# genome-vendor/bsmap

Hardware: AMD Instinct MI355X
Metric: aligned reads/sec (whole node), 2x150 bp hg38 WGBS -v 6 -s 16 (higher is better)
Workload: dtype u32; 1 GPU; C3: 2x150(->144) bp PE WGBS vs hg38-sized synthetic genome, -s 16 -v 6 -I 4 -m 28 -x 500; genome_bp=3088269832, index_entries=1475952693, parallelism=read-sharded x1, batches_in_flight=2, exact_mode=False, resident_ring_steps=4, records_flagged_BSX_F_LIMIT=0

## Files before the change

### bsmap_amd/csrc/bsx_align.hip

```cpp
#include "bsx_internal.h"
#include "bsx_dev.h"
#include "bsx_kernel_args.h"

namespace {

typedef unsigned long long u64;

struct __attribute__((packed, aligned(4))) U4 { uint32_t a, b, c, d; };
struct __attribute__((packed, aligned(4))) U2 { uint32_t a, b; };

#ifndef BSX_MAIN_NT
#define BSX_MAIN_NT 0
#endif
#ifndef BSX_MAIN_PREFETCH
#define BSX_MAIN_PREFETCH 1
#endif
typedef uint32_t v4u_a4 __attribute__((ext_vector_type(4), aligned(4)));
typedef uint32_t v2u_a4 __attribute__((ext_vector_type(2), aligned(4)));
__device__ __forceinline__ U4 ldm4(const uint32_t *p)
{
#if BSX_MAIN_NT
    const v4u_a4 v = __builtin_nontemporal_load(reinterpret_cast<const v4u_a4 *>(p));
    return U4{v.x, v.y, v.z, v.w};
#else
// ... 2199 lines not shown
    __shared__ uint32_t TAB[BSX_HSCAN_WPB][4][32];
    __shared__ uint2 PT[BSX_HSCAN_WPB][HP_PAIRS * 32];
    __shared__ uint2 QBUF[BSX_HSCAN_WPB][HP_QCAP];
    const int lane = threadIdx.x & 63, wv = (int)rfl(threadIdx.x >> 6);
    const uint32_t n_tasks = min(*H.n_tasks, H.task_cap);
    const uint32_t nvb = (n_tasks + BSX_HSCAN_WPB - 1) / BSX_HSCAN_WPB;
    for (uint32_t vb = blockIdx.x;; vb += gridDim.x) {
        uint32_t b_;
        const int st_ = bsx_order_block(vb, nvb, H.xcd_map, b_);
        if (st_ == 2) break;
        if (st_ == 1) continue;
        const uint32_t slot = b_ * BSX_HSCAN_WPB + (uint32_t)wv;
        if (slot < n_tasks) hp_task<STATS>(A, H, H.order ? rfl(H.order[slot]) : slot, lane, TAB[wv], PT[wv], QBUF[wv]);
        wave_fence();
    }
}

#ifndef HG_WPB
#define HG_WPB 1
#endif
#ifndef HG_R
#define HG_R 64u
#endif
static_assert(HG_R == 16u || HG_R == 32u || HG_R == 48u || HG_R == 64u, "a lane per member: 64 at most, and whole quarters of a segment");
#ifndef HG_XCD_DIV
#define HG_XCD_DIV (HG_R > 16u ? 2u : 1u)
#endif
#ifndef HG_C
#define HG_C 4
#endif
#ifndef HG_BIG
#define HG_BIG (HG_R > 32u ? 33u : 1u)
#endif
#ifndef HG_PREFETCH
#define HG_PREFETCH 0
#endif
#ifndef HG_EXIT
#define HG_EXIT 15
#endif
#ifndef BSX_HSAME_WAVES
#define BSX_HSAME_WAVES 4
#endif
#ifndef HG_D
#define HG_D 2
#endif
#ifndef HG_ROWPF
#define HG_ROWPF 0
// ... 354 lines not shown
        uint32_t tid = 0, th = 0, tc0 = 0, tn = 0, key = 0, hh = 0, flags = 0, tx = 0, tw = 0;
        if ((uint32_t)lane < K) {
            tid = H.order[slot + lane];
            const HTask tk = H.tasks[tid];
            th = tk.h; tc0 = tk.c0; tn = tk.n; key = tk.key; hh = tk.sub_h; flags = tk.flags; tx = tk.pad[0]; tw = tk.pad[1];
        }
        const uint32_t n0 = rfl(tn), f0 = rfl(flags);
        if (n0 == 0) {
            if ((uint32_t)lane < K) { HTaskOut *o = &H.tout[tid]; o->count = 0; o->overflow = 0; o->acc[0] = o->acc[1] = o->acc[2] = o->acc[3] = 0; o->c0 = 0; o->n = 0; }
        } else if (f0 & 4u) {
            if (((f0 >> 8) & 15u) == 3u) hs_group<3, true, STATS>(A, H, L, lane, wv, K, tid, th, tc0, rfl(key), n0, rfl(hh), hh, f0, rfl(tx), rfl(tw));
            else hs_group<0, true, STATS>(A, H, L, lane, wv, K, tid, th, tc0, rfl(key), n0, rfl(hh), hh, f0, rfl(tx), rfl(tw));
        }
        else if (K > 1) {
            if (((f0 >> 8) & 15u) == 5u) hs_group<5, false, STATS>(A, H, L, lane, wv, K, tid, th, tc0, rfl(key), n0, rfl(hh), hh, f0, 0u, 0u);
            else if (((f0 >> 8) & 15u) == 4u) hs_group<4, false, STATS>(A, H, L, lane, wv, K, tid, th, tc0, rfl(key), n0, rfl(hh), hh, f0, 0u, 0u);
            else hs_group<0, false, STATS>(A, H, L, lane, wv, K, tid, th, tc0, rfl(key), n0, rfl(hh), hh, f0, 0u, 0u);
        }
        else hp_task<STATS>(A, H, rfl(tid), lane, L.W[wv].one.TAB, L.W[wv].one.PT, L.W[wv].one.Q);
        wave_fence();
    }
}

__global__ __launch_bounds__(256) void k_task_groups(const HTask *tasks, const uint32_t *n_tasks_ptr, uint32_t cap, uint32_t *order, uint32_t *ghead, uint32_t *glist, uint32_t D, uint32_t Rg)
{
    const int lane = threadIdx.x & 63;
    const uint32_t n_tasks = min(*n_tasks_ptr, cap);
    for (uint32_t s0 = (blockIdx.x * 4u + (threadIdx.x >> 6)) * 64u; s0 < n_tasks; s0 += gridDim.x * 256u) {
        const uint32_t nj = min(64u, n_tasks - s0);
        uint32_t tid = 0, tn = 0, key = 0, hh = 0, flags = 0, tx = 0, tw = 0;
        if ((uint32_t)lane < nj) {
            tid = order[s0 + lane];
            const HTask tk = tasks[tid];
            tn = tk.n; key = tk.key; hh = tk.sub_h; flags = tk.flags; tx = tk.pad[0]; tw = tk.pad[1];
        }
        u64 todo = bsx_ballot((uint32_t)lane < nj);
        uint32_t off = 0, head = 0, dst = 0;
        while (todo) {
            const uint32_t i0 = (uint32_t)__builtin_ctzll(todo);
            const uint32_t n0 = rl_u(tn, i0), f0 = rl_u(flags, i0), key0 = rl_u(key, i0), h0 = rl_u(hh, i0), tx0 = rl_u(tx, i0), tw0 = rl_u(tw, i0);
            const bool pending = (todo >> lane) & 1;
            u64 mem = 1ull << i0;
            if (n0 == 0) mem = bsx_ballot(pending && tn == 0);
            else if (f0 & 2u) {
                const uint32_t Dg = (!(f0 & 4u) && ((f0 >> 8) & 15u) == 5u) ? D : 0u;
                const bool win = pending && tn == n0 && key == key0 && flags == f0 && tx == tx0 && tw == tw0;
                uint32_t hmin = h0;
                if (Dg) {
                    uint32_t v = win && ((hh ^ h0) & 31u) == 0 ? hh ^ 0x80000000u : 0xffffffffu;
#pragma unroll
                    for (int o = 32; o; o >>= 1) v = min(v, (uint32_t)__shfl_xor(v, o));
                    hmin = v ^ 0x80000000u;
                }
                const uint32_t dh = hh - hmin;
                mem = 0;
                uint32_t Kg = 0;
                for (uint32_t dd = 0; dd <= Dg && Kg < Rg; dd++) {
                    const bool same = win && dh == 32u * dd;
                    u64 md = bsx_ballot(same);
                    if (Kg + (uint32_t)__builtin_popcountll(md) > Rg) md = bsx_ballot(same && Kg + (uint32_t)__builtin_popcountll(md & lanemask_lt(lane)) < Rg);
                    if ((md >> lane) & 1) dst = off + Kg + (uint32_t)__builtin_popcountll(md & lanemask_lt(lane));
                    mem |= md; Kg += (uint32_t)__builtin_popcountll(md);
                }
            }
            const uint32_t K = (uint32_t)__builtin_popcountll(mem);
            if (!(n0 != 0 && (f0 & 2u)) && ((mem >> lane) & 1)) dst = off + (uint32_t)__builtin_popcountll(mem & lanemask_lt(lane));
            if ((uint32_t)lane == off) head = K;
            off += K; todo &= ~mem;
        }
        if ((uint32_t)lane < nj) { order[s0 + dst] = tid; ghead[s0 + lane] = head; }
        const u64 hb = bsx_ballot(head >= HG_BIG), hs = bsx_ballot(head != 0 && head < HG_BIG);
        uint32_t base = 0;
        if (lane == 0 && hb) base = atomicAdd(&glist[cap], (uint32_t)__builtin_popcountll(hb));
        if (lane == 1 && hs) base = atomicAdd(&glist[cap + 1], (uint32_t)__builtin_popcountll(hs));
        const uint32_t base_b = rl_u(base, 0), base_s = rl_u(base, 1);
        if (head >= HG_BIG) glist[base_b + (uint32_t)__builtin_popcountll(hb & lanemask_lt(lane))] = s0 + (uint32_t)lane;
        else if (head != 0) glist[cap - 1u - (base_s + (uint32_t)__builtin_popcountll(hs & lanemask_lt(lane)))] = s0 + (uint32_t)lane;
    }
}

#define HS_SHARE 16u
#ifndef BSX_HSHARED_W3
#define BSX_HSHARED_W3 1
#endif
#ifndef BSX_HSHARED_C2
#define BSX_HSHARED_C2 1
#endif
#ifndef BSX_HSHARED_WAVES
#define BSX_HSHARED_WAVES 5
#endif
struct SharedChunk { uint32_t wd[12]; uint32_t pm1, strand; bool valid; };

__device__ __forceinline__ U2 shared_entry(const U2 *__restrict__ ent2, uint32_t idx, bool in_range)
{
    U2 e; e.a = 0xFFFFFFFFu; e.b = 0;
    if (in_range) e = ent2[idx];
    return e;
}
template <int NWR, bool LDS_CHR>
__device__ __forceinline__ SharedChunk shared_gather(const U2 e, bool in_range, uint32_t h, uint32_t tag_xor, uint32_t tag_want, const uint32_t *anch_lds,
// ... 390 lines not shown
}
__global__ __launch_bounds__(256) void k_task_order(const HTask *tasks, const uint32_t *n_tasks_ptr, uint32_t cap, uint32_t shift, uint32_t n_bins, uint32_t spread, const uint32_t *bstart,
                                                     const uint32_t *chunk_tot, uint32_t n_chunks, const uint32_t *rank, uint32_t *order)
{
    __shared__ uint32_t cstart[1024];
    const uint32_t n = min(*n_tasks_ptr, cap);
    if (n == 0) return;
    for (uint32_t i = threadIdx.x; i < 1024; i += 256) cstart[i] = i < n_chunks ? chunk_tot[i] : 0u;
    __syncthreads();
    for (uint32_t o = 1; o < 1024; o <<= 1) {
        uint32_t t[4];
        for (int k = 0; k < 4; k++) { const uint32_t i = threadIdx.x + 256 * k; t[k] = i >= o ? cstart[i - o] : 0u; }
        __syncthreads();
        for (int k = 0; k < 4; k++) cstart[threadIdx.x + 256 * k] += t[k];
        __syncthreads();
    }
    for (uint32_t i = blockIdx.x * 256 + threadIdx.x; i < n; i += gridDim.x * 256) {
        const uint32_t b = task_bin(tasks[i], shift, n_bins, spread), c = b / BIN_CHUNK;
        order[(c ? cstart[c - 1] : 0u) + bstart[b] + rank[i]] = i;
    }
}
}

uint32_t bsx_bin_chunks(uint32_t n_bins) { return (n_bins + BIN_CHUNK - 1) / BIN_CHUNK; }

void bsx_launch_task_order(const HeavyArgsRaw &R, uint32_t shift, uint32_t n_bins, uint32_t *bins, uint32_t *bstart, uint32_t *chunk_tot, uint32_t *rank, uint32_t *order,
                           uint32_t *zero_blk, hipStream_t stream, uint32_t spread, bool groups, uint32_t same_d, uint32_t same_r)
{
    const uint32_t grid = std::max(1u, std::min(512u, (R.task_cap + 255u) / 256u)), n_chunks = bsx_bin_chunks(n_bins);
    hipLaunchKernelGGL(k_task_bins, dim3(std::max(1u, std::min(256u, (R.task_cap + 1023u) / 1024u))), dim3(256), 0, stream, (const HTask *)R.tasks, R.n_tasks, R.task_cap, shift, n_bins, spread, bins, rank, zero_blk);
    hipLaunchKernelGGL(k_bin_scan, dim3(n_chunks), dim3(256), 0, stream, R.n_tasks, bins, bstart, chunk_tot, n_bins, groups ? R.glist + R.task_cap : (uint32_t *)nullptr);
    hipLaunchKernelGGL(k_task_order, dim3(grid), dim3(256), 0, stream, (const HTask *)R.tasks, R.n_tasks, R.task_cap, shift, n_bins, spread, bstart, chunk_tot, n_chunks, rank, order);
    if (groups) hipLaunchKernelGGL(k_task_groups, dim3(std::max(1u, std::min(1024u, (R.task_cap + 255u) / 256u))), dim3(256), 0, stream, (const HTask *)R.tasks, R.n_tasks, R.task_cap, order, rank, R.glist, std::min<uint32_t>(same_d, HG_D), same_r ? std::min<uint32_t>(same_r, HG_R) : HG_R);
}

namespace {
__device__ __forceinline__ unsigned long long sig_of(const HTask &tk, bool with_h)
{
    unsigned long long x = ((unsigned long long)tk.key << 32) ^ ((unsigned long long)tk.n << 9) ^ (tk.flags & 1u) ^ (with_h ? (unsigned long long)tk.sub_h * 0x9E3779B97F4A7C15ull : 0ull);
    x ^= x >> 29; x *= 0xBF58476D1CE4E5B9ull; x ^= x >> 32;
    return x | 1ull;
}
__global__ __launch_bounds__(256) void k_sig_count(const HTask *tasks, const uint32_t *n_tasks_ptr, uint32_t cap, unsigned long long *tab, uint32_t mask, int with_h)
{
    const uint32_t n = min(*n_tasks_ptr, cap);
    for (uint32_t i = blockIdx.x * 256 + threadIdx.x; i < n; i += gridDim.x * 256) {
        const HTask tk = tasks[i];
        if (!tk.n || !(tk.flags & 2u)) continue;
        const unsigned long long sg = sig_of(tk, with_h != 0);
        for (uint32_t slot = (uint32_t)(sg >> 20) & mask;; slot = (slot + 1) & mask) {
            const unsigned long long prev = atomicCAS(&tab[2 * (size_t)slot], 0ull, sg);
            if (prev == 0ull || prev == sg) { atomicAdd(&tab[2 * (size_t)slot + 1], 1ull); break; }
        }
    }
}
__global__ __launch_bounds__(256) void k_sig_hist(const HTask *tasks, const uint32_t *n_tasks_ptr, uint32_t cap, const unsigned long long *tab, uint32_t mask, int with_h, unsigned long long *hist)
// ... 36 lines not shown
    }
}
__global__ __launch_bounds__(256) void k_sigc_count(const HTask *tasks, const uint32_t *n_tasks_ptr, uint32_t cap, unsigned long long *tab, uint32_t mask, uint32_t D, int pass, unsigned long long *hist)
{
    const uint32_t n = min(*n_tasks_ptr, cap);
    for (uint32_t i = blockIdx.x * 256 + threadIdx.x; i < n; i += gridDim.x * 256) {
        const HTask tk = tasks[i];
        if (!tk.n) continue;
        uint32_t k = 31;
        if (tk.flags & 2u) {
            const unsigned long long sg = sigc_of(tk);
            uint32_t slot = (uint32_t)(sg >> 20) & mask, probes = 0;
            while (tab[2 * (size_t)slot] != sg && probes <= mask) { slot = (slot + 1) & mask; probes++; }
            if (probes > mask) continue;
            const unsigned long long w = tab[2 * (size_t)slot + 1];
            const bool within = sigc_class(tk) - (0x0fffffffu - (uint32_t)(w & 0xffffffffull)) <= D;
            if (!pass) { if (within) atomicAdd(&tab[2 * (size_t)slot + 1], 1ull << 32); continue; }
            const uint32_t r = (uint32_t)(w >> 32);
            k = !within ? 30u : r <= 1 ? 0u : 32u - (uint32_t)__builtin_clz(r - 1u);
        }
        if (pass) { atomicAdd(&hist[k], (unsigned long long)tk.n); atomicAdd(&hist[32 + k], 1ull); }
    }
}
const int SIG_KINDS = 5;
unsigned long long *g_sig_tab = nullptr, *g_sig_hist = nullptr;
const uint32_t SIG_SLOTS = 1u << 23;
}

void bsx_sig_hist_pass(const HeavyArgsRaw &R, hipStream_t stream)
{
    if (!g_sig_tab) {
        if (hipMalloc((void **)&g_sig_tab, (size_t)SIG_SLOTS * 16) != hipSuccess || hipMalloc((void **)&g_sig_hist, SIG_KINDS * 64 * 8) != hipSuccess) { g_sig_tab = nullptr; return; }
        (void)hipMemsetAsync(g_sig_hist, 0, SIG_KINDS * 64 * 8, stream);
    }
    for (int with_h = 0; with_h < 2; with_h++) {
        (void)hipMemsetAsync(g_sig_tab, 0, (size_t)SIG_SLOTS * 16, stream);
        hipLaunchKernelGGL(k_sig_count, dim3(1024), dim3(256), 0, stream, (const HTask *)R.tasks, R.n_tasks, R.task_cap, g_sig_tab, SIG_SLOTS - 1, with_h);
        hipLaunchKernelGGL(k_sig_hist, dim3(1024), dim3(256), 0, stream, (const HTask *)R.tasks, R.n_tasks, R.task_cap, g_sig_tab, SIG_SLOTS - 1, with_h, g_sig_hist + 64 * with_h);
    }
    for (int kind = 2; kind < SIG_KINDS; kind++) {
        const uint32_t D = kind == 2 ? 1u : kind == 3 ? 2u : 4u;
        (void)hipMemsetAsync(g_sig_tab, 0, (size_t)SIG_SLOTS * 16, stream);
        hipLaunchKernelGGL(k_sigc_min, dim3(1024), dim3(256), 0, stream, (const HTask *)R.tasks, R.n_tasks, R.task_cap, g_sig_tab, SIG_SLOTS - 1);
        for (int pass = 0; pass < 2; pass++)
            hipLaunchKernelGGL(k_sigc_count, dim3(1024), dim3(256), 0, stream, (const HTask *)R.tasks, R.n_tasks, R.task_cap, g_sig_tab, SIG_SLOTS - 1, D, pass, g_sig_hist + 64 * kind);
    }
}

void bsx_sig_hist_report(void)
{
    if (!g_sig_tab) return;
    unsigned long long h[SIG_KINDS * 64];
    if (hipDeviceSynchronize() != hipSuccess || hipMemcpy(h, g_sig_hist, sizeof h, hipMemcpyDeviceToHost) != hipSuccess) return;
    static const char *const kind_name[SIG_KINDS] = {"", " and offset", " and offset mod 32, offset / 32 within 1 of the smallest", " and offset mod 32, offset / 32 within 2 of the smallest",
                                                     " and offset mod 32, offset / 32 within 4 of the smallest"};
    for (int with_h = 0; with_h < SIG_KINDS; with_h++) {
        unsigned long long tot = 0, tt = 0;
        for (int k = 0; k < 32; k++) { tot += h[64 * with_h + k]; tt += h[64 * with_h + 32 + k]; }
        fprintf(stderr, "[sighist] same window%s: candidates %llu tasks %llu\n", kind_name[with_h], tot, tt);
        for (int k = 0; k < 32; k++)
            if (h[64 * with_h + 32 + k])
                fprintf(stderr, "[sighist]   %s %-6u cand %.4f tasks %.4f\n", k == 31 ? "spanning" : k == 30 && with_h >= 2 ? "beyond" : "R <=", k == 31 || (k == 30 && with_h >= 2) ? 0u : 1u << k, (double)h[64 * with_h + k] / (double)std::max(1ull, tot), (double)h[64 * with_h + 32 + k] / (double)std::max(1ull, tt));
    }
    (void)hipMemset(g_sig_hist, 0, SIG_KINDS * 64 * 8);
}

void bsx_sector_pass(const bsx_ref *r, hipStream_t stream)
{
#ifdef BSX_SECTOR_STATS
    const uint32_t n_words = (uint32_t)(((uint64_t)r->plane_rc_off * 2 / 64 + 31) / 32 + 64);
    static uint32_t *bits = nullptr;
    if (!bits) {
        if (hipMalloc((void **)&bits, (size_t)n_words * 4) != hipSuccess) return;
        (void)hipMemset(bits, 0, (size_t)n_words * 4);
        (void)hipMemcpyToSymbol(HIP_SYMBOL(g_sector_bits), &bits, sizeof(bits));
        return;
    }
    hipLaunchKernelGGL(k_sector_pop, dim3(1024), dim3(256), 0, stream, n_words);
#else
    (void)r; (void)stream;
#endif
}
void bsx_sector_report(void)
{
#ifdef BSX_SECTOR_STATS
    unsigned long long t = 0, d = 0, p = 0;
    if (hipDeviceSynchronize() != hipSuccess) return;
// ... 29 lines not shown
```

### bsmap_amd/csrc/bsx_api.hip

```cpp
#include <fcntl.h>
#include <sys/mman.h>
#include <sys/stat.h>
#include <unistd.h>
#include <time.h>

#include <cstdio>
#include <cstdlib>
#include <cstring>
#include <fstream>
#include <cmath>
#include <vector>

#include "bsx_internal.h"
#include "bsx_kernel_args.h"

static int g_waves_per_cu = 0;
static int g_heavy_threshold = 0;

extern "C" int bsx_set_waves_per_cu(int w) { g_waves_per_cu = w; return BSX_OK; }
extern "C" int bsx_set_heavy_threshold(int t) { g_heavy_threshold = t < 0 ? 0 : t; return BSX_OK; }
static uint32_t heavy_threshold_for(const bsx_params &p) { return g_heavy_threshold > 0 ? (uint32_t)g_heavy_threshold : (p.rrbs ? 2048u : 32768u); }
static bool g_user_limits = false;
static uint32_t g_hcap = 24576, g_task_cap = 1048576;
extern "C" int bsx_set_heavy_limits(uint32_t units_per_round, uint32_t task_pool)
// ... 234 lines not shown
    uint32_t tail_tasks = 16384, tail_grid_tasks = 4096;
    uint32_t bin_shift = 0, n_bins = 1;
    hipEvent_t ev_sync = nullptr, ev_wait = nullptr;
    std::vector<hipEvent_t> scan_ev;
    size_t scan_ev_used = 0;
    hipEvent_t ev0 = nullptr, ev1 = nullptr;
    uint8_t *d_seq[2] = {nullptr, nullptr}, *d_qual[2] = {nullptr, nullptr};
    uint64_t *d_off[2] = {nullptr, nullptr};
    size_t seq_cap[2] = {0, 0};
    bsx_hit *d_hits = nullptr;
    bsx_pair *d_pairs = nullptr;
    bsx_class_counts *d_cc[2] = {nullptr, nullptr};
    uint16_t *d_npairs = nullptr;
    uint8_t *d_scratch = nullptr, *d_dbg = nullptr;
    uint32_t *d_cycles = nullptr;
    uint32_t *d_heavy_list = nullptr, *d_heavy_count = nullptr;
    uint8_t *d_hstate = nullptr, *d_hslabs = nullptr, *d_htasks = nullptr, *d_htout = nullptr;
    uint32_t *d_hactive[2] = {nullptr, nullptr}, *d_hcnt = nullptr;
    uint32_t hcap = 0, task_cap = 0;
    bool sig_hist = false;
    bool same_kernel = false;
    uint32_t same_d = 0;
    uint32_t same_r = 0;
    bool sector_stats = false;
    uint32_t xcd_map = 128;
    uint32_t *h_pinned = nullptr;
    int n_cu = 0;
    uint32_t last_heavy = 0, last_heavy_iters = 0, last_redo = 0;
    size_t scratch_bytes = 0;
    uint32_t *d_queue = nullptr;
    uint64_t *d_counters = nullptr, *d_scan_stats = nullptr;
    uint64_t slab_bytes = 0, hslab_bytes = 0;
    uint32_t *d_redo = nullptr;
    uint32_t rowcap = 0, hkcap = 0;
    int grid_blocks = 0;
    std::vector<hipEvent_t> ctrl_ev;
    size_t ctrl_ev_used = 0;
    hipEvent_t ev_align = nullptr;
    bool stage_timing = false;
    uint32_t *d_ah_pool = nullptr;
    uint64_t ah_cap = 0;
    uint64_t *d_ah_ctl = nullptr;
    bsx_span *d_ah_spans = nullptr;
    uint32_t run_first = 0, run_units = 0;
    bool ah_ran = false;
    bool ran = false;
// ... 135 lines not shown
    }
    if (!b->d_heavy_list) {
        const BatchPlan pl = plan_batch(b->ref->P, b->paired, b->max_units, b->ref->n_entries, prop.multiProcessorCount, blocks_per_cu, b->n_groups, b->debug != 0);
        b->hcap = pl.hcap; b->task_cap = pl.task_cap;
        HIP_TRY(hipMalloc((void **)&b->d_heavy_list, ((size_t)b->max_units + 1) * 4));
        HIP_TRY(hipMalloc((void **)&b->d_heavy_count, 256));
        HIP_TRY(hipHostMalloc((void **)&b->h_pinned, 1024, hipHostMallocDefault));
        HIP_TRY(hipMalloc((void **)&b->d_redo, ((size_t)b->max_units + 1) * 4));
        HIP_TRY(hipMalloc((void **)&b->d_hcnt, (size_t)BSX_MAX_GROUPS * 2 * BSX_HCNT_BLOCK * 4));
        b->bin_shift = pl.bin_shift; b->n_bins = pl.n_bins;
        auto free_pools = [&]() {
            void **ptrs[] = {(void **)&b->d_hstate, (void **)&b->d_hslabs, (void **)&b->d_htasks, (void **)&b->d_htout, (void **)&b->d_hactive[0], (void **)&b->d_hactive[1]};
            for (void **q : ptrs) { if (*q) (void)hipFree(*q); *q = nullptr; }
            for (int g = 0; g < b->n_groups; g++) {
                bsx_batch::Group &q = b->grp[g];
                void **gp[] = {(void **)&q.d_bins, (void **)&q.d_bstart, (void **)&q.d_chunk_tot, (void **)&q.d_rank, (void **)&q.d_order, (void **)&q.d_glist};
                for (void **x : gp) { if (*x) (void)hipFree(*x); *x = nullptr; }
            }
        };
        const int same_env0 = getenv("BSX_SAME") ? atoi(getenv("BSX_SAME")) : 1;
        const bool same_kernel = b->same_kernel = b->ref->P.rrbs ? same_env0 == 2 : same_env0 != 0;
        b->same_d = getenv("BSX_SAME_D") ? (uint32_t)std::min<long>(std::max<long>(0, atol(getenv("BSX_SAME_D"))), (long)bsx_same_d_max()) : bsx_same_d_max();
        b->same_r = getenv("BSX_SAME_R") ? (uint32_t)std::min<long>(std::max<long>(1, atol(getenv("BSX_SAME_R"))), (long)bsx_same_r_max()) : bsx_same_r_max();
        auto alloc_pools = [&]() -> hipError_t {
            hipError_t e;
#define POOL_TRY(x) do { if ((e = (x)) != hipSuccess) return e; } while (0)
            POOL_TRY(hipMalloc((void **)&b->d_hstate, (size_t)b->hcap * bsx_hstate_bytes()));
            POOL_TRY(hipMalloc((void **)&b->d_hslabs, (size_t)b->hcap * b->hslab_bytes));
            POOL_TRY(hipMalloc((void **)&b->d_htasks, (size_t)b->task_cap * bsx_htask_bytes()));
            POOL_TRY(hipMalloc((void **)&b->d_htout, (size_t)b->task_cap * bsx_htaskout_bytes()));
            for (int k = 0; k < 2; k++) POOL_TRY(hipMalloc((void **)&b->d_hactive[k], (size_t)b->hcap * 4));
            const uint32_t tcap = b->task_cap / (uint32_t)b->n_groups;
            for (int g = 0; g < b->n_groups; g++) {
                bsx_batch::Group &q = b->grp[g];
                POOL_TRY(hipMalloc((void **)&q.d_bins, (size_t)b->n_bins * 4));
                POOL_TRY(hipMalloc((void **)&q.d_bstart, (size_t)b->n_bins * 4));
                POOL_TRY(hipMalloc((void **)&q.d_chunk_tot, (size_t)bsx_bin_chunks(b->n_bins) * 4));
                POOL_TRY(hipMalloc((void **)&q.d_rank, (size_t)tcap * 4));
                POOL_TRY(hipMalloc((void **)&q.d_order, (size_t)tcap * 4));
                if (same_kernel) POOL_TRY(hipMalloc((void **)&q.d_glist, ((size_t)tcap + 4) * 4));
            }
#undef POOL_TRY
            return hipSuccess;
        };
        const uint64_t reserve = g_pool_reserve ? g_pool_reserve : ((4ull << 30) + pl.scratch_bytes + pl.per_unit_bytes);
        for (int attempt = 0;; attempt++) {
// ... 371 lines not shown
        const uint32_t n_rounds = (n_heavy + b->hcap - 1) / b->hcap, per_round = n_rounds ? (n_heavy + n_rounds - 1) / n_rounds : 0;
        for (uint32_t base = 0; base < n_heavy; base += per_round) {
            const uint32_t n_round = std::min(per_round, n_heavy - base);
            Group G[BSX_MAX_GROUPS];
            HIP_TRY(hipEventRecord(b->ev_sync, b->stream));
            auto enqueue_pass = [&](int g) -> int {
                Group &q = G[g];
                bsx_batch::Group &hw = b->grp[g];
                uint32_t *in = q.blk[q.cur], *out = q.blk[q.cur ^ 1];
                const bool fresh = q.passes == 0;
                if (fresh) {
                    HIP_TRY(hipStreamWaitEvent(hw.s_ctrl, b->ev_sync, 0));
                    HIP_TRY(hipMemsetAsync(out, 0, (size_t)BSX_HCNT_BLOCK * 4, hw.s_ctrl));
                } else HIP_TRY(hipStreamWaitEvent(hw.s_ctrl, hw.ev_scan, 0));
                q.H.active_in = b->d_hactive[q.cur] + q.H.hidx_base; q.H.active_out = b->d_hactive[q.cur ^ 1] + q.H.hidx_base;
                q.H.n_active_in_ptr = in; q.H.n_active_in = q.n0; q.H.n_active_out = out; q.H.n_tasks = out + BSX_HCNT_TASKS; q.H.queue = out + BSX_HCNT_QUEUE;
                q.H.fresh = fresh ? 1 : 0;
                while (b->stage_timing && b->ctrl_ev_used + 3 > b->ctrl_ev.size()) { hipEvent_t ev_new = nullptr; HIP_TRY(hipEventCreate(&ev_new)); b->ctrl_ev.push_back(ev_new); }
                if (b->stage_timing) HIP_TRY(hipEventRecord(b->ctrl_ev[b->ctrl_ev_used], hw.s_ctrl));
                bsx_launch_hctrl(A, q.H, b->paired, (int)std::min<uint32_t>((q.n0 + 3) / 4, (uint32_t)b->n_cu * b->hctrl_blocks_per_cu), hw.s_ctrl, ah);
                HIP_TRY(hipGetLastError());
                if (b->stage_timing) HIP_TRY(hipEventRecord(b->ctrl_ev[b->ctrl_ev_used + 1], hw.s_ctrl));
                q.H.order = hw.d_order; q.H.xcd_map = b->xcd_map; q.H.ghead = hw.d_rank; q.H.glist = hw.d_glist;
                bsx_launch_task_order(q.H, b->bin_shift, b->n_bins, hw.d_bins, hw.d_bstart, hw.d_chunk_tot, hw.d_rank, hw.d_order, in, hw.s_ctrl, spread, same_scan, b->same_d, b->same_r);
                if (b->stage_timing) { HIP_TRY(hipEventRecord(b->ctrl_ev[b->ctrl_ev_used + 2], hw.s_ctrl)); b->ctrl_ev_used += 3; }
                if (b->sig_hist) bsx_sig_hist_pass(q.H, hw.s_ctrl);
                hipStream_t s_scan = b->stream;
                if (q.tail) s_scan = hw.s_ctrl;
                else {
                    HIP_TRY(hipEventRecord(hw.ev_ctrl, hw.s_ctrl));
                    HIP_TRY(hipStreamWaitEvent(b->stream, hw.ev_ctrl, 0));
                }
                if (b->scan_ev_used + 2 > b->scan_ev.size()) {
                    hipEvent_t e0, e1;
                    HIP_TRY(hipEventCreate(&e0)); HIP_TRY(hipEventCreate(&e1));
                    b->scan_ev.push_back(e0); b->scan_ev.push_back(e1);
                }
                HIP_TRY(hipEventRecord(b->scan_ev[b->scan_ev_used], s_scan));
                if (same_scan) bsx_launch_hscan_same(A, q.H, s_scan, q.tail ? b->tail_grid_tasks : 0);
                else if (shared_scan) bsx_launch_hscan_shared(A, q.H, s_scan, q.tail ? b->tail_grid_tasks : 0);
                else bsx_launch_hscan(A, q.H, s_scan, q.tail ? b->tail_grid_tasks : 0);
                HIP_TRY(hipGetLastError());
                if (b->sector_stats) bsx_sector_pass(b->ref, s_scan);
                HIP_TRY(hipEventRecord(b->scan_ev[b->scan_ev_used + 1], s_scan));
                b->scan_ev_used += 2;
                HIP_TRY(hipEventRecord(hw.ev_scan, s_scan));
                q.cur ^= 1; q.passes++;
                b->last_heavy_iters++;
                return BSX_OK;
// ... 147 lines not shown
        std::vector<uint16_t> tmp((size_t)b->n_units * 32);
        HIP_TRY(hipMemcpy(tmp.data(), b->d_npairs, tmp.size() * 2, hipMemcpyDeviceToHost));
        for (uint32_t u = 0; u < b->n_units; u++) memcpy(n_pairs31 + (size_t)u * 31, tmp.data() + (size_t)u * 32, 62);
    }
    return BSX_OK;
}

extern "C" int bsx_batch_counters(bsx_batch *b, uint64_t c[BSX_N_COUNTERS])
{
    if (!b || !c) return BSX_ERR_ARG;
    HIP_TRY(hipSetDevice(b->ref->device));
    HIP_TRY(stream_wait(b));
    HIP_TRY(hipMemcpy(c, b->d_counters, BSX_N_COUNTERS * 8, hipMemcpyDeviceToHost));
    uint64_t sh[64 * 8];
    HIP_TRY(hipMemcpy(sh, b->d_scan_stats, sizeof(sh), hipMemcpyDeviceToHost));
#ifdef BSX_SCAN_WORDS
    for (int i = 0; i < 64; i++) { for (int k = 0; k < 4; k++) c[7 + k] += sh[i * 8 + k]; c[15] += sh[i * 8 + 4]; }
    if (sh[5])
        fprintf(stderr, "[scanwords] 129-160 nt: %llu (read, 64-candidate chunk) evaluations, %llu words, mean %.3f words per evaluation\n",
                (unsigned long long)sh[5], (unsigned long long)sh[6], (double)sh[6] / (double)sh[5]);
#else
    uint64_t dg[3] = {0, 0, 0};
    for (int i = 0; i < 64; i++) { for (int k = 0; k < 4; k++) c[7 + k] += sh[i * 8 + k]; c[15] += sh[i * 8 + 4]; for (int k = 0; k < 3; k++) dg[k] += sh[i * 8 + 5 + k]; }
    if (b->sig_hist && c[15])
        fprintf(stderr, "[sighist] scan kernel: %.4f of the candidates in groups, mean group %.2f reads, in groups of >= 4 %.4f; evaluations of a read whose words and threshold equal an earlier member's of its group: %.4f of all\n", (double)c[15] / (double)std::max<uint64_t>(1, c[7]),
                (double)dg[0] / (double)c[15], (double)dg[1] / (double)c[7], (double)dg[2] / (double)c[7]);
#endif
    return BSX_OK;
}
extern "C" int bsx_batch_reset_counters(bsx_batch *b)
{
    if (!b) return BSX_ERR_ARG;
    HIP_TRY(hipSetDevice(b->ref->device));
    HIP_TRY(hipMemsetAsync(b->d_counters, 0, BSX_N_COUNTERS * 8, b->stream));
    HIP_TRY(hipMemsetAsync(b->d_scan_stats, 0, 64 * 64, b->stream));
    HIP_TRY(stream_wait(b));
    return BSX_OK;
}

extern "C" int bsx_batch_download_reads(bsx_batch *b, int mate, char *seqs, uint64_t *off)
{
    if (!b || mate < 0 || mate > (b->paired ? 1 : 0) || !off) return BSX_ERR_ARG;
    HIP_TRY(hipSetDevice(b->ref->device));
    HIP_TRY(stream_wait(b));
    HIP_TRY(hipMemcpy(off, b->d_off[mate], ((size_t)b->n_units + 1) * 8, hipMemcpyDeviceToHost));
    if (seqs) HIP_TRY(hipMemcpy(seqs, b->d_seq[mate], off[b->n_units], hipMemcpyDeviceToHost));
    return BSX_OK;
}

// ... 192 lines not shown
```

### bsmap_amd/csrc/bsx_kernel_args.h

```cpp
#pragma once
#include "bsx_internal.h"

struct AlignArgs {
    DevParams P;
    uint32_t n_units, first_index;
    uint32_t first_unit;
    int32_t debug;
    uint32_t rowcap;
    uint32_t kcap, hbits;
    uint32_t hkcap, hhbits;
    uint64_t hslab_bytes;
    uint32_t *redo_list, *redo_count;
    const uint32_t *unit_list;
    const uint8_t *seq[2];
    const uint64_t *off[2];
    const uint8_t *qual[2];
    bsx_hit *hits_out;
    bsx_pair *pairs_out;
    bsx_class_counts *cc[2];
    uint16_t *npairs_out;
    uint8_t *scratch;
    uint64_t slab_bytes;
    uint32_t work_counters;
    uint32_t heavy_threshold;
// ... 42 lines not shown
    uint32_t *n_tasks;
    uint32_t *queue;
    const uint32_t *n_active_in_ptr;
    uint32_t n_active_in, task_cap, fresh, list_base, hidx_base;
    const uint32_t *order;
    uint32_t xcd_map;
    const uint32_t *ghead;
    uint32_t *glist;
};

void bsx_launch_align(const AlignArgs &A, int paired, int grid_blocks, hipStream_t stream, const AllHitsArgs *ah = nullptr);
void bsx_launch_align_ah(const AlignArgs &A, int paired, int grid_blocks, hipStream_t stream, const AllHitsArgs &X);
void bsx_launch_hctrl_ah(const AlignArgs &A, const HeavyArgsRaw &H, int paired, int grid_blocks, hipStream_t stream, const AllHitsArgs &X);
void bsx_launch_leak(const AlignArgs &A, int paired, int n_cu, bool with_meta, bool resolve, void *final_out, hipStream_t stream);
size_t bsx_leakrec_bytes(void);
size_t bsx_leakstate_bytes(void);
uint32_t bsx_leak_blk(void);
void bsx_launch_hctrl(const AlignArgs &A, const HeavyArgsRaw &H, int paired, int grid_blocks, hipStream_t stream, const AllHitsArgs *ah = nullptr);
void bsx_launch_hscan(const AlignArgs &A, const HeavyArgsRaw &H, hipStream_t stream, uint32_t max_tasks = 0);
void bsx_launch_hscan_same(const AlignArgs &A, const HeavyArgsRaw &H, hipStream_t stream, uint32_t max_tasks = 0);
void bsx_launch_hscan_shared(const AlignArgs &A, const HeavyArgsRaw &H, hipStream_t stream, uint32_t max_tasks = 0);
uint32_t bsx_bin_chunks(uint32_t n_bins);
void bsx_launch_task_order(const HeavyArgsRaw &H, uint32_t shift, uint32_t n_bins, uint32_t *bins, uint32_t *bstart, uint32_t *chunk_tot, uint32_t *rank, uint32_t *order,
                           uint32_t *zero_blk, hipStream_t stream, uint32_t spread = 0, bool groups = false, uint32_t same_d = 0, uint32_t same_r = 0);
uint32_t bsx_same_d_max(void);
uint32_t bsx_same_r_max(void);
void bsx_sig_hist_pass(const HeavyArgsRaw &H, hipStream_t stream);
void bsx_sig_hist_report(void);
void bsx_sector_pass(const bsx_ref *r, hipStream_t stream);
void bsx_sector_report(void);
size_t bsx_hstate_bytes(void);
size_t bsx_htask_bytes(void);
size_t bsx_htaskout_bytes(void);
int bsx_align_occupancy(int paired);
int bsx_hctrl_occupancy(int paired);
```

Measured before the change: 41.35 million reads/s.

## Form same-signature task groups by sorting tiles of tasks in LDS

The task grouping kernel no longer groups only within 64-task wave windows by repeated ballots. Each block now loads a tile of up to 1024 tasks into LDS, bitonic-sorts them by key, a hash of the signature and sub_h, and then cuts runs of equal signature into groups with a shared helper that caps group size and frame distance. The aim is to find more and larger groups so the downstream heavy scan shares more fetches. The cost is more LDS, a full bitonic sort with many block barriers per tile, and a hash that could collide, though collisions are rechecked before a run is joined. Optional diagnostics count fetches per group and signature sets split by tile borders.

```diff
diff --git a/bsmap_amd/csrc/bsx_align.hip b/bsmap_amd/csrc/bsx_align.hip
--- a/bsmap_amd/csrc/bsx_align.hip
+++ b/bsmap_amd/csrc/bsx_align.hip
@@ -1,5 +1,6 @@
 #include "bsx_internal.h"
 #include "bsx_dev.h"
+#include "bsx_groups.h"
 #include "bsx_kernel_args.h"
 
 namespace {
@@ -2245,7 +2246,7 @@
 #ifndef HG_R
 #define HG_R 64u
 #endif
-static_assert(HG_R == 16u || HG_R == 32u || HG_R == 48u || HG_R == 64u, "a lane per member: 64 at most, and whole quarters of a segment");
+static_assert(HG_R == 16u || HG_R == 32u || HG_R == 48u || HG_R == 64u, "a lane per member: 64 at most");
 #ifndef HG_XCD_DIV
 #define HG_XCD_DIV (HG_R > 16u ? 2u : 1u)
 #endif
@@ -2646,60 +2647,114 @@
     }
 }
 
-__global__ __launch_bounds__(256) void k_task_groups(const HTask *tasks, const uint32_t *n_tasks_ptr, uint32_t cap, uint32_t *order, uint32_t *ghead, uint32_t *glist, uint32_t D, uint32_t Rg)
-{
+#ifndef HG_TILE
+#define HG_TILE 1024u
+#endif
+#define HG_TILE_MAX 2048u
+static_assert(HG_TILE >= 64u && HG_TILE <= HG_TILE_MAX && (HG_TILE & (HG_TILE - 1u)) == 0, "a power of two of whole waves");
+__device__ __forceinline__ bool tg_less(const uint4 &a, const uint4 &b)
+{
+    if (a.x != b.x) return a.x < b.x;
+    if (a.y != b.y) return a.y < b.y;
+    if (a.z != b.z) return a.z < b.z;
+    return a.w < b.w;
+}
+__device__ __forceinline__ bool tg_same_run(const HTask &a, const HTask &b)
+{
+    if (a.n == 0 || b.n == 0) return a.n == b.n;
+    return (a.flags & 2u) && a.flags == b.flags && a.key == b.key && a.n == b.n && a.pad[0] == b.pad[0] && a.pad[1] == b.pad[1] && ((a.sub_h ^ b.sub_h) & 31u) == 0;
+}
+__global__ __launch_bounds__(256) void k_task_groups(const HTask *tasks, const uint32_t *n_tasks_ptr, uint32_t cap, uint32_t *order, uint32_t *ghead, uint32_t *glist, uint32_t D, uint32_t Rg,
+                                                     uint32_t T, uint32_t big)
+{
+    extern __shared__ uint4 tg_lds[];
+    uint4 *K = tg_lds;
+    uint32_t *head = (uint32_t *)(K + T);
+    u64 *brk = (u64 *)(head + T);
+    uint32_t *cnt = (uint32_t *)(brk + HG_TILE_MAX / 64u);
     const int lane = threadIdx.x & 63;
+    const uint32_t wv = threadIdx.x >> 6, n_ch = T >> 6;
     const uint32_t n_tasks = min(*n_tasks_ptr, cap);
-    for (uint32_t s0 = (blockIdx.x * 4u + (threadIdx.x >> 6)) * 64u; s0 < n_tasks; s0 += gridDim.x * 256u) {
-        const uint32_t nj = min(64u, n_tasks - s0);
-        uint32_t tid = 0, tn = 0, key = 0, hh = 0, flags = 0, tx = 0, tw = 0;
-        if ((uint32_t)lane < nj) {
-            tid = order[s0 + lane];
-            const HTask tk = tasks[tid];
-            tn = tk.n; key = tk.key; hh = tk.sub_h; flags = tk.flags; tx = tk.pad[0]; tw = tk.pad[1];
-        }
-        u64 todo = bsx_ballot((uint32_t)lane < nj);
-        uint32_t off = 0, head = 0, dst = 0;
-        while (todo) {
-            const uint32_t i0 = (uint32_t)__builtin_ctzll(todo);
-            const uint32_t n0 = rl_u(tn, i0), f0 = rl_u(flags, i0), key0 = rl_u(key, i0), h0 = rl_u(hh, i0), tx0 = rl_u(tx, i0), tw0 = rl_u(tw, i0);
-            const bool pending = (todo >> lane) & 1;
-            u64 mem = 1ull << i0;
-            if (n0 == 0) mem = bsx_ballot(pending && tn == 0);
-            else if (f0 & 2u) {
-                const uint32_t Dg = (!(f0 & 4u) && ((f0 >> 8) & 15u) == 5u) ? D : 0u;
-                const bool win = pending && tn == n0 && key == key0 && flags == f0 && tx == tx0 && tw == tw0;
-                uint32_t hmin = h0;
-                if (Dg) {
-                    uint32_t v = win && ((hh ^ h0) & 31u) == 0 ? hh ^ 0x80000000u : 0xffffffffu;
-#pragma unroll
-                    for (int o = 32; o; o >>= 1) v = min(v, (uint32_t)__shfl_xor(v, o));
-                    hmin = v ^ 0x80000000u;
+    for (uint32_t s0 = blockIdx.x * T; s0 < n_tasks; s0 += gridDim.x * T) {
+        const uint32_t nj = min(T, n_tasks - s0);
+        for (uint32_t i = threadIdx.x; i < T; i += 256u) {
+            uint4 k = make_uint4(0xffffffffu, 0xffffffffu, 0xffffffffu, 0xffffffffu);
+            if (i < nj) {
+                const uint32_t tid = order[s0 + i];
+                const HTask tk = tasks[tid];
+                if (tk.n == 0) k = make_uint4(0xffffffffu, 0xfffffffeu, 0u, tid);
+                else {
+                    uint32_t hs = tk.n * 0x9E3779B1u ^ tk.flags * 0x85EBCA6Bu ^ tk.pad[0] * 0xC2B2AE35u ^ tk.pad[1] * 0x27D4EB2Fu;
+                    hs ^= hs >> 15; hs *= 0x2C1B3C6Du; hs ^= hs >> 13;
+                    k = make_uint4(tk.key, (hs & ~31u) | (tk.sub_h & 31u), tk.sub_h ^ 0x80000000u, tid);
                 }
-                const uint32_t dh = hh - hmin;
-                mem = 0;
-                uint32_t Kg = 0;
-                for (uint32_t dd = 0; dd <= Dg && Kg < Rg; dd++) {
-                    const bool same = win && dh == 32u * dd;
-                    u64 md = bsx_ballot(same);
-                    if (Kg + (uint32_t)__builtin_popcountll(md) > Rg) md = bsx_ballot(same && Kg + (uint32_t)__builtin_popcountll(md & lanemask_lt(lane)) < Rg);
-                    if ((md >> lane) & 1) dst = off + Kg + (uint32_t)__builtin_popcountll(md & lanemask_lt(lane));
-                    mem |= md; Kg += (uint32_t)__builtin_popcountll(md);
+            }
+            K[i] = k;
+        }
+        __syncthreads();
+        for (uint32_t kk = 2; kk <= T; kk <<= 1)
+            for (uint32_t j = kk >> 1; j; j >>= 1) {
+                for (uint32_t t = threadIdx.x; t < (T >> 1); t += 256u) {
+                    const uint32_t i = 2u * t - (t & (j - 1u)), l = i + j;
+                    const uint4 a = K[i], b = K[l];
+                    if (tg_less(b, a) == ((i & kk) == 0)) { K[i] = b; K[l] = a; }
                 }
-            }
-            const uint32_t K = (uint32_t)__builtin_popcountll(mem);
-            if (!(n0 != 0 && (f0 & 2u)) && ((mem >> lane) & 1)) dst = off + (uint32_t)__builtin_popcountll(mem & lanemask_lt(lane));
-            if ((uint32_t)lane == off) head = K;
-            off += K; todo &= ~mem;
-        }
-        if ((uint32_t)lane < nj) { order[s0 + dst] = tid; ghead[s0 + lane] = head; }
-        const u64 hb = bsx_ballot(head >= HG_BIG), hs = bsx_ballot(head != 0 && head < HG_BIG);
-        uint32_t base = 0;
-        if (lane == 0 && hb) base = atomicAdd(&glist[cap], (uint32_t)__builtin_popcountll(hb));
-        if (lane == 1 && hs) base = atomicAdd(&glist[cap + 1], (uint32_t)__builtin_popcountll(hs));
-        const uint32_t base_b = rl_u(base, 0), base_s = rl_u(base, 1);
-        if (head >= HG_BIG) glist[base_b + (uint32_t)__builtin_popcountll(hb & lanemask_lt(lane))] = s0 + (uint32_t)lane;
-        else if (head != 0) glist[cap - 1u - (base_s + (uint32_t)__builtin_popcountll(hs & lanemask_lt(lane)))] = s0 + (uint32_t)lane;
+                __syncthreads();
+            }
+        uint32_t info[HG_TILE_MAX / 256u];
+#pragma unroll
+        for (uint32_t m = 0; m < HG_TILE_MAX / 256u; m++) {
+            const uint32_t c = wv + 4u * m, i = c * 64u + (uint32_t)lane;
+            info[m] = 0;
+            if (c >= n_ch) continue;
+            bool start = false;
+            if (i < nj) {
+                const uint4 k = K[i];
+                const HTask tk = tasks[k.w];
+                start = true;
+                if (i) {
+                    const uint4 kp = K[i - 1u];
+                    if (kp.x == k.x && kp.y == k.y) start = !tg_same_run(tasks[kp.w], tk);
+                }
+                const uint32_t Dg = (!(tk.flags & 4u) && ((tk.flags >> 8) & 15u) == 5u) ? D : 0u;
+                if (start) info[m] = 1u | (tk.n == 0 ? 64u << 8 : !(tk.flags & 2u) ? 1u << 8 : Dg << 1 | Rg << 8);
+            }
+            const u64 bm = bsx_ballot(start);
+            if (lane == 0) brk[c] = bm;
+        }
+        __syncthreads();
+#pragma unroll
+        for (uint32_t m = 0; m < HG_TILE_MAX / 256u; m++) {
+            if (!info[m]) continue;
+            const uint32_t i = (wv + 4u * m) * 64u + (uint32_t)lane;
+            uint32_t c = i >> 6;
+            u64 w = brk[c] & ~((2ull << (i & 63u)) - 1ull);
+            while (!w && ++c < n_ch) w = brk[c];
+            const uint32_t e = w ? c * 64u + (uint32_t)__builtin_ctzll(w) : nj;
+            bsx_group_cut(&K[i].z, 4u, e - i, (info[m] >> 1) & 127u, info[m] >> 8, head + i, 1u);
+        }
+        __syncthreads();
+        for (uint32_t c = wv; c < n_ch; c += 4u) {
+            const uint32_t i = c * 64u + (uint32_t)lane, hd = i < nj ? head[i] : 0u;
+            if (i < nj) { order[s0 + i] = K[i].w; ghead[s0 + i] = hd; }
+            const u64 hb = bsx_ballot(hd >= big), hsm = bsx_ballot(hd != 0 && hd < big);
+            if (lane == 0) { cnt[c] = (uint32_t)__builtin_popcountll(hb); cnt[32u + c] = (uint32_t)__builtin_popcountll(hsm); }
+        }
+        __syncthreads();
+        if (threadIdx.x < 2u) {
+            uint32_t *q = cnt + 32u * threadIdx.x, tot = 0;
+            for (uint32_t c = 0; c < n_ch; c++) tot += q[c];
+            uint32_t run = tot ? atomicAdd(&glist[cap + threadIdx.x], tot) : 0u;
+            for (uint32_t c = 0; c < n_ch; c++) { const uint32_t v = q[c]; q[c] = run; run += v; }
+        }
+        __syncthreads();
+        for (uint32_t c = wv; c < n_ch; c += 4u) {
+            const uint32_t i = c * 64u + (uint32_t)lane, hd = i < nj ? head[i] : 0u;
+            const u64 hb = bsx_ballot(hd >= big), hsm = bsx_ballot(hd != 0 && hd < big);
+            if (hd >= big) glist[cnt[c] + (uint32_t)__builtin_popcountll(hb & lanemask_lt(lane))] = s0 + i;
+            else if (hd != 0) glist[cap - 1u - (cnt[32u + c] + (uint32_t)__builtin_popcountll(hsm & lanemask_lt(lane)))] = s0 + i;
+        }
+        __syncthreads();
     }
 }
 
@@ -3136,16 +3191,27 @@
 }
 }
 
+uint32_t bsx_group_tile(uint32_t tile)
+{
+    uint32_t T = 64u;
+    while (T < HG_TILE_MAX && T < (tile ? tile : HG_TILE)) T <<= 1;
+    return T;
+}
 uint32_t bsx_bin_chunks(uint32_t n_bins) { return (n_bins + BIN_CHUNK - 1) / BIN_CHUNK; }
 
 void bsx_launch_task_order(const HeavyArgsRaw &R, uint32_t shift, uint32_t n_bins, uint32_t *bins, uint32_t *bstart, uint32_t *chunk_tot, uint32_t *rank, uint32_t *order,
-                           uint32_t *zero_blk, hipStream_t stream, uint32_t spread, bool groups, uint32_t same_d, uint32_t same_r)
+                           uint32_t *zero_blk, hipStream_t stream, uint32_t spread, bool groups, uint32_t same_d, uint32_t same_r, uint32_t tile, uint32_t big)
 {
     const uint32_t grid = std::max(1u, std::min(512u, (R.task_cap + 255u) / 256u)), n_chunks = bsx_bin_chunks(n_bins);
     hipLaunchKernelGGL(k_task_bins, dim3(std::max(1u, std::min(256u, (R.task_cap + 1023u) / 1024u))), dim3(256), 0, stream, (const HTask *)R.tasks, R.n_tasks, R.task_cap, shift, n_bins, spread, bins, rank, zero_blk);
     hipLaunchKernelGGL(k_bin_scan, dim3(n_chunks), dim3(256), 0, stream, R.n_tasks, bins, bstart, chunk_tot, n_bins, groups ? R.glist + R.task_cap : (uint32_t *)nullptr);
     hipLaunchKernelGGL(k_task_order, dim3(grid), dim3(256), 0, stream, (const HTask *)R.tasks, R.n_tasks, R.task_cap, shift, n_bins, spread, bstart, chunk_tot, n_chunks, rank, order);
-    if (groups) hipLaunchKernelGGL(k_task_groups, dim3(std::max(1u, std::min(1024u, (R.task_cap + 255u) / 256u))), dim3(256), 0, stream, (const HTask *)R.tasks, R.n_tasks, R.task_cap, order, rank, R.glist, std::min<uint32_t>(same_d, HG_D), same_r ? std::min<uint32_t>(same_r, HG_R) : HG_R);
+    if (groups) {
+        const uint32_t T = bsx_group_tile(tile);
+        const size_t lds = (size_t)T * 20u + HG_TILE_MAX / 64u * 8u + 64u * 4u;
+        hipLaunchKernelGGL(k_task_groups, dim3(std::max(1u, std::min(1024u, (R.task_cap + T - 1u) / T))), dim3(256), lds, stream, (const HTask *)R.tasks, R.n_tasks, R.task_cap, order, rank, R.glist,
+                           std::min<uint32_t>(same_d, HG_D), same_r ? std::min<uint32_t>(same_r, HG_R) : HG_R, T, big ? std::min<uint32_t>(big, HG_R + 1u) : HG_BIG);
+    }
 }
 
 namespace {
@@ -3228,16 +3294,48 @@
         if (pass) { atomicAdd(&hist[k], (unsigned long long)tk.n); atomicAdd(&hist[32 + k], 1ull); }
     }
 }
+__global__ __launch_bounds__(256) void k_group_fetches(const HTask *tasks, uint32_t cap, const uint32_t *order, const uint32_t *ghead, const uint32_t *glist, unsigned long long *st)
+{
+    const uint32_t n_big = min(glist[cap], cap), n_groups = min(n_big + glist[cap + 1], cap);
+    unsigned long long ev = 0, ch = 0;
+    for (uint32_t g = blockIdx.x * 256 + threadIdx.x; g < n_groups; g += gridDim.x * 256) {
+        const uint32_t slot = glist[g < n_big ? g : cap - 1u - (g - n_big)], n = tasks[order[slot]].n;
+        ev += (unsigned long long)ghead[slot] * n; ch += (n + 63u) / 64u;
+    }
+    if (ev) { atomicAdd(&st[0], ev); atomicAdd(&st[1], ch); }
+}
+__global__ __launch_bounds__(256) void k_sigc_tiles(const HTask *tasks, const uint32_t *n_tasks_ptr, uint32_t cap, const uint32_t *order, unsigned long long *tab, uint32_t mask, uint32_t T, int pass, unsigned long long *st)
+{
+    const uint32_t n = min(*n_tasks_ptr, cap);
+    for (uint32_t s = blockIdx.x * 256 + threadIdx.x; s < n; s += gridDim.x * 256) {
+        const HTask tk = tasks[order[s]];
+        if (!tk.n || !(tk.flags & 2u)) continue;
+        const unsigned long long sg = sigc_of(tk);
+        if (!pass) {
+            for (uint32_t slot = (uint32_t)(sg >> 20) & mask;; slot = (slot + 1) & mask) {
+                const unsigned long long prev = atomicCAS(&tab[2 * (size_t)slot], 0ull, sg);
+                if (prev == 0ull || prev == sg) { atomicOr(&tab[2 * (size_t)slot + 1], 1ull << ((s / T) & 63u)); break; }
+            }
+            continue;
+        }
+        uint32_t slot = (uint32_t)(sg >> 20) & mask, probes = 0;
+        while (tab[2 * (size_t)slot] != sg && probes <= mask) { slot = (slot + 1) & mask; probes++; }
+        if (probes > mask) continue;
+        const unsigned long long w = tab[2 * (size_t)slot + 1];
+        atomicAdd(&st[2], (unsigned long long)tk.n);
+        if (w & (w - 1ull)) atomicAdd(&st[3], (unsigned long long)tk.n);
+    }
+}
 const int SIG_KINDS = 5;
 unsigned long long *g_sig_tab = nullptr, *g_sig_hist = nullptr;
 const uint32_t SIG_SLOTS = 1u << 23;
 }
 
-void bsx_sig_hist_pass(const HeavyArgsRaw &R, hipStream_t stream)
+void bsx_sig_hist_pass(const HeavyArgsRaw &R, hipStream_t stream, bool groups, uint32_t tile)
 {
     if (!g_sig_tab) {
-        if (hipMalloc((void **)&g_sig_tab, (size_t)SIG_SLOTS * 16) != hipSuccess || hipMalloc((void **)&g_sig_hist, SIG_KINDS * 64 * 8) != hipSuccess) { g_sig_tab = nullptr; return; }
-        (void)hipMemsetAsync(g_sig_hist, 0, SIG_KINDS * 64 * 8, stream);
+        if (hipMalloc((void **)&g_sig_tab, (size_t)SIG_SLOTS * 16) != hipSuccess || hipMalloc((void **)&g_sig_hist, (SIG_KINDS * 64 + 4) * 8) != hipSuccess) { g_sig_tab = nullptr; return; }
+        (void)hipMemsetAsync(g_sig_hist, 0, (SIG_KINDS * 64 + 4) * 8, stream);
     }
     for (int with_h = 0; with_h < 2; with_h++) {
         (void)hipMemsetAsync(g_sig_tab, 0, (size_t)SIG_SLOTS * 16, stream);
@@ -3251,6 +3349,17 @@
         for (int pass = 0; pass < 2; pass++)
             hipLaunchKernelGGL(k_sigc_count, dim3(1024), dim3(256), 0, stream, (const HTask *)R.tasks, R.n_tasks, R.task_cap, g_sig_tab, SIG_SLOTS - 1, D, pass, g_sig_hist + 64 * kind);
     }
+    if (groups) {
+        hipLaunchKernelGGL(k_group_fetches, dim3(1024), dim3(256), 0, stream, (const HTask *)R.tasks, R.task_cap, R.order, R.ghead, R.glist, g_sig_hist + 64 * SIG_KINDS);
+        (void)hipMemsetAsync(g_sig_tab, 0, (size_t)SIG_SLOTS * 16, stream);
+        for (int pass = 0; pass < 2; pass++)
+            hipLaunchKernelGGL(k_sigc_tiles, dim3(1024), dim3(256), 0, stream, (const HTask *)R.tasks, R.n_tasks, R.task_cap, R.order, g_sig_tab, SIG_SLOTS - 1, bsx_group_tile(tile), pass, g_sig_hist + 64 * SIG_KINDS);
+    }
+}
+
+bool bsx_sig_group_stats(unsigned long long st[4])
+{
+    return g_sig_tab && hipDeviceSynchronize() == hipSuccess && hipMemcpy(st, g_sig_hist + 64 * SIG_KINDS, 32, hipMemcpyDeviceToHost) == hipSuccess;
 }
 
 void bsx_sig_hist_report(void)
@@ -3268,7 +3377,7 @@
             if (h[64 * with_h + 32 + k])
                 fprintf(stderr, "[sighist]   %s %-6u cand %.4f tasks %.4f\n", k == 31 ? "spanning" : k == 30 && with_h >= 2 ? "beyond" : "R <=", k == 31 || (k == 30 && with_h >= 2) ? 0u : 1u << k, (double)h[64 * with_h + k] / (double)std::max(1ull, tot), (double)h[64 * with_h + 32 + k] / (double)std::max(1ull, tt));
     }
-    (void)hipMemset(g_sig_hist, 0, SIG_KINDS * 64 * 8);
+    (void)hipMemset(g_sig_hist, 0, (SIG_KINDS * 64 + 4) * 8);
 }
 
 void bsx_sector_pass(const bsx_ref *r, hipStream_t stream)
diff --git a/bsmap_amd/csrc/bsx_api.hip b/bsmap_amd/csrc/bsx_api.hip
--- a/bsmap_amd/csrc/bsx_api.hip
+++ b/bsmap_amd/csrc/bsx_api.hip
@@ -280,6 +280,8 @@
     bool same_kernel = false;
     uint32_t same_d = 0;
     uint32_t same_r = 0;
+    uint32_t group_tile = 0;
+    uint32_t group_big = 0;
     bool sector_stats = false;
     uint32_t xcd_map = 128;
     uint32_t *h_pinned = nullptr;
@@ -461,6 +463,8 @@
         const bool same_kernel = b->same_kernel = b->ref->P.rrbs ? same_env0 == 2 : same_env0 != 0;
         b->same_d = getenv("BSX_SAME_D") ? (uint32_t)std::min<long>(std::max<long>(0, atol(getenv("BSX_SAME_D"))), (long)bsx_same_d_max()) : bsx_same_d_max();
         b->same_r = getenv("BSX_SAME_R") ? (uint32_t)std::min<long>(std::max<long>(1, atol(getenv("BSX_SAME_R"))), (long)bsx_same_r_max()) : bsx_same_r_max();
+        b->group_tile = getenv("BSX_GROUP_TILE") ? (uint32_t)std::max<long>(0, atol(getenv("BSX_GROUP_TILE"))) : 0u;
+        b->group_big = getenv("BSX_GROUP_BIG") ? (uint32_t)std::max<long>(0, atol(getenv("BSX_GROUP_BIG"))) : 0u;
         auto alloc_pools = [&]() -> hipError_t {
             hipError_t e;
 #define POOL_TRY(x) do { if ((e = (x)) != hipSuccess) return e; } while (0)
@@ -878,9 +882,9 @@
                 HIP_TRY(hipGetLastError());
                 if (b->stage_timing) HIP_TRY(hipEventRecord(b->ctrl_ev[b->ctrl_ev_used + 1], hw.s_ctrl));
                 q.H.order = hw.d_order; q.H.xcd_map = b->xcd_map; q.H.ghead = hw.d_rank; q.H.glist = hw.d_glist;
-                bsx_launch_task_order(q.H, b->bin_shift, b->n_bins, hw.d_bins, hw.d_bstart, hw.d_chunk_tot, hw.d_rank, hw.d_order, in, hw.s_ctrl, spread, same_scan, b->same_d, b->same_r);
+                bsx_launch_task_order(q.H, b->bin_shift, b->n_bins, hw.d_bins, hw.d_bstart, hw.d_chunk_tot, hw.d_rank, hw.d_order, in, hw.s_ctrl, spread, same_scan, b->same_d, b->same_r, b->group_tile, b->group_big);
                 if (b->stage_timing) { HIP_TRY(hipEventRecord(b->ctrl_ev[b->ctrl_ev_used + 2], hw.s_ctrl)); b->ctrl_ev_used += 3; }
-                if (b->sig_hist) bsx_sig_hist_pass(q.H, hw.s_ctrl);
+                if (b->sig_hist) bsx_sig_hist_pass(q.H, hw.s_ctrl, same_scan, b->group_tile);
                 hipStream_t s_scan = b->stream;
                 if (q.tail) s_scan = hw.s_ctrl;
                 else {
@@ -1074,9 +1078,14 @@
 #else
     uint64_t dg[3] = {0, 0, 0};
     for (int i = 0; i < 64; i++) { for (int k = 0; k < 4; k++) c[7 + k] += sh[i * 8 + k]; c[15] += sh[i * 8 + 4]; for (int k = 0; k < 3; k++) dg[k] += sh[i * 8 + 5 + k]; }
-    if (b->sig_hist && c[15])
-        fprintf(stderr, "[sighist] scan kernel: %.4f of the candidates in groups, mean group %.2f reads, in groups of >= 4 %.4f; evaluations of a read whose words and threshold equal an earlier member's of its group: %.4f of all\n", (double)c[15] / (double)std::max<uint64_t>(1, c[7]),
-                (double)dg[0] / (double)c[15], (double)dg[1] / (double)c[7], (double)dg[2] / (double)c[7]);
+    if (b->sig_hist && c[15]) {
+        unsigned long long gs[4] = {0, 0, 0, 0};
+        (void)bsx_sig_group_stats(gs);
+        fprintf(stderr, "[sighist] scan kernel: %.4f of the candidates in groups, mean group %.2f reads, in groups of >= 4 %.4f; evaluations of a read whose words and threshold equal an earlier member's of its group: %.4f of all"
+                "; reads per fetch %.2f (%llu evaluations, %llu group chunks), candidates in sets that a tile border cut %.4f\n", (double)c[15] / (double)std::max<uint64_t>(1, c[7]),
+                (double)dg[0] / (double)c[15], (double)dg[1] / (double)c[7], (double)dg[2] / (double)c[7],
+                (double)gs[0] / (64.0 * (double)std::max(1ull, gs[1])), gs[0], gs[1], (double)gs[3] / (double)std::max(1ull, gs[2]));
+    }
 #endif
     return BSX_OK;
 }
diff --git a/bsmap_amd/csrc/bsx_groups.h b/bsmap_amd/csrc/bsx_groups.h
--- /dev/null
+++ b/bsmap_amd/csrc/bsx_groups.h
@@ -0,0 +1,22 @@
+#pragma once
+#include <hip/hip_runtime.h>
+#include <stdint.h>
+
+__host__ __device__ inline uint32_t bsx_group_cut(const uint32_t *off, uint32_t stride, uint32_t n, uint32_t D, uint32_t Rg, uint32_t *head, uint32_t hstride)
+{
+    if (Rg == 0) Rg = 1;
+    uint32_t groups = 0;
+    for (uint32_t p = 0; p < n; groups++) {
+        const uint32_t frame = off[(size_t)p * stride];
+        uint32_t lo = p + 1, hi = n;
+        while (lo < hi) {
+            const uint32_t mid = lo + ((hi - lo) >> 1);
+            if (off[(size_t)mid * stride] - frame <= 32u * D) lo = mid + 1; else hi = mid;
+        }
+        const uint32_t N = lo - p, G = (N + Rg - 1u) / Rg, k = (N + G - 1u) / G;
+        head[(size_t)p * hstride] = k;
+        for (uint32_t j = 1; j < k; j++) head[(size_t)(p + j) * hstride] = 0;
+        p += k;
+    }
+    return groups;
+}
diff --git a/bsmap_amd/csrc/bsx_kernel_args.h b/bsmap_amd/csrc/bsx_kernel_args.h
--- a/bsmap_amd/csrc/bsx_kernel_args.h
+++ b/bsmap_amd/csrc/bsx_kernel_args.h
@@ -88,10 +88,12 @@
 void bsx_launch_hscan_shared(const AlignArgs &A, const HeavyArgsRaw &H, hipStream_t stream, uint32_t max_tasks = 0);
 uint32_t bsx_bin_chunks(uint32_t n_bins);
 void bsx_launch_task_order(const HeavyArgsRaw &H, uint32_t shift, uint32_t n_bins, uint32_t *bins, uint32_t *bstart, uint32_t *chunk_tot, uint32_t *rank, uint32_t *order,
-                           uint32_t *zero_blk, hipStream_t stream, uint32_t spread = 0, bool groups = false, uint32_t same_d = 0, uint32_t same_r = 0);
+                           uint32_t *zero_blk, hipStream_t stream, uint32_t spread = 0, bool groups = false, uint32_t same_d = 0, uint32_t same_r = 0, uint32_t tile = 0, uint32_t big = 0);
 uint32_t bsx_same_d_max(void);
 uint32_t bsx_same_r_max(void);
-void bsx_sig_hist_pass(const HeavyArgsRaw &H, hipStream_t stream);
+void bsx_sig_hist_pass(const HeavyArgsRaw &H, hipStream_t stream, bool groups = false, uint32_t tile = 0);
+bool bsx_sig_group_stats(unsigned long long st[4]);
+uint32_t bsx_group_tile(uint32_t tile);
 void bsx_sig_hist_report(void);
 void bsx_sector_pass(const bsx_ref *r, hipStream_t stream);
 void bsx_sector_report(void);
```

Measured after the change: 43.54 million reads/s (median of 6 runs). +5.3%, better.
